# WojciechMula/pyahocorasick

Measured on NVIDIA H100. Metric: haystack GB/s, higher is better.
Workload: dtype u8

## Files before the change

### pyahocorasick_b200/csrc/acb_device.cu

```cuda
#include "acb_internal.h"
#include "acb_hash.h"

#include <cuda_runtime.h>
#include <cub/device/device_radix_sort.cuh>
#include <cub/device/device_scan.cuh>
#include <cub/device/device_select.cuh>

#include <algorithm>
#include <atomic>
#include <mutex>
#include <chrono>
#include <cstdio>
#include <cstdlib>
#include <cstring>
#include <exception>
#include <new>
#include <vector>

#define CUDA_TRY(expr)                                                                       \
    do {                                                                                     \
        cudaError_t _e = (expr);                                                             \
        if (_e != cudaSuccess) {                                                             \
            acb_set_error("CUDA error %s at %s:%d: %s", cudaGetErrorName(_e), __FILE__,      \
                          __LINE__, cudaGetErrorString(_e));                                 \
// ... 103 lines not shown
        hs = h * p.stride_bytes;
        he = hs + p.stride_bytes;
    } else {
        long long lo = 0, hi = p.n_hay;
        while (hi - lo > 1) {
            long long mid = (lo + hi) >> 1;
            if (__ldg(p.offsets + mid) <= q) lo = mid; else hi = mid;
        }
        h = lo;
        hs = __ldg(p.offsets + lo);
        he = __ldg(p.offsets + lo + 1);
    }
}

struct WarpStage {
    acb_match *buf;
    int *cnt;
};

__device__ __forceinline__ void emit(const ScanParams &p, const WarpStage &ws, int32_t h, int32_t e, int32_t k) {
    acb_match m;
    m.hay_id = h;
    m.end_index = e;
    m.key_id = k;
    int slot;
    asm volatile("atom.shared.add.u32 %0, [%1], 1;" : "=r"(slot) : "r"((uint32_t)__cvta_generic_to_shared(ws.cnt)) : "memory");
    if (slot < kStageCap) {
        ws.buf[slot] = m;
    } else {
        unsigned long long g = atomicAdd(p.count, 1ULL);
        if (g < (unsigned long long)p.cap) p.out[g] = m;
    }
}

__device__ __forceinline__ void flush_stage(const ScanParams &p, const WarpStage &ws, int lane) {
    __syncwarp();
    int n = *ws.cnt;
    if (n > kStageCap) n = kStageCap;
    if (n > 0) {
        unsigned long long base = 0;
        if (lane == 0) base = atomicAdd(p.count, (unsigned long long)n);
        base = __shfl_sync(kFull, base, 0);
#pragma unroll
        for (int i = lane; i < kStageCap; i += 32)
            if (i < n && base + i < (unsigned long long)p.cap) p.out[base + i] = ws.buf[i];
    }
    __syncwarp();
    if (lane == 0) *ws.cnt = 0;
    __syncwarp();
}

__device__ __forceinline__ void walk_from(const ScanParams &p, const WarpStage &ws, long long start,
                                          long long h, long long hs, long long he) {
    const int L = p.L;
    int32_t st = 0;
    for (long long i = start; i < he; ++i) {
        int c = __ldg(p.cls + p.hay[i]);
        int32_t nx = __ldg(p.gto + (long long)c * p.S + st);
        if (nx < 0) break;
        st = nx & kIdMask;
        if (nx & kTermBit) {
            int32_t k = __ldg(p.key_of + st);
            emit(p, ws, (int32_t)h, (int32_t)((i - hs + 1) / L - 1), k);
        }
    }
}

template <class P>
__device__ __forceinline__ void load_text(const P &p, long long x, uint32_t (&w)[6]) {
    const long long x0 = x & ~3LL;
    if (x0 + 24 <= p.total) {
        const uint32_t *a = reinterpret_cast<const uint32_t *>(p.hay + x0);
#pragma unroll
        for (int i = 0; i < 6; i++) w[i] = __ldg(a + i);
    } else {
#pragma unroll
        for (int i = 0; i < 6; i++) w[i] = load_word(p.hay, x0 + 4 * i, p.total);
    }
}

__device__ __forceinline__ bool text_equals(const uint32_t (&w)[6], long long x, int n, const uint32_t kw[5]) {
    const int sh = (int)(x & 3) * 8;
    uint32_t diff = 0;
#pragma unroll
    for (int i = 0; i < 5; i++) {
        uint32_t t = __funnelshift_r(w[i], w[i + 1], sh);
        int nb = n - 4 * i;
        uint32_t mask = nb >= 4 ? 0xffffffffu : (nb <= 0 ? 0u : ((1u << (8 * nb)) - 1u));
        diff |= (t ^ kw[i]) & mask;
    }
    return diff == 0;
}


__device__ __forceinline__ unsigned long long mul_wide(uint32_t a, uint32_t b) {
    unsigned long long d;
    asm("mul.wide.u32 %0, %1, %2;" : "=l"(d) : "r"(a), "r"(b));
    return d;
}
__device__ __forceinline__ unsigned long long mad_wide(uint32_t a, uint32_t b, unsigned long long c) {
    unsigned long long d;
    asm("mad.wide.u32 %0, %1, %2, %3;" : "=l"(d) : "r"(a), "r"(b), "l"(c));
    return d;
}
__device__ __forceinline__ uint32_t lds32(uint32_t saddr) {
    uint32_t v;
    asm volatile("ld.shared.u32 %0, [%1];" : "=r"(v) : "r"(saddr));
    return v;
}
__device__ __forceinline__ uint2 lds64(uint32_t saddr) {
    uint2 v;
    asm volatile("ld.shared.v2.u32 {%0, %1}, [%2];" : "=r"(v.x), "=r"(v.y) : "r"(saddr) : "memory");
    return v;
}
__device__ __forceinline__ uint32_t lds16(uint32_t saddr) {
    uint32_t v;
    asm volatile("{ .reg .u16 h; ld.shared.u16 h, [%1]; cvt.u32.u16 %0, h; }" : "=r"(v) : "r"(saddr) : "memory");
    return v;
}
__device__ __forceinline__ void sts16(uint32_t saddr, uint32_t v) {
    asm volatile("{ .reg .u16 h; cvt.u16.u32 h, %1; st.shared.u16 [%0], h; }" :: "r"(saddr), "r"(v) : "memory");
}
__device__ __forceinline__ uint4 lds128(uint32_t saddr) {
    uint4 v;
    asm volatile("ld.shared.v4.u32 {%0, %1, %2, %3}, [%4];" : "=r"(v.x), "=r"(v.y), "=r"(v.z), "=r"(v.w) : "r"(saddr));
    return v;
}
__device__ __forceinline__ uint32_t lds_bitmap(uint32_t saddr) {
    uint32_t v;
    asm("ld.shared.u32 %0, [%1];" : "=r"(v) : "r"(saddr));
    return v;
}

__device__ __forceinline__ void mbar_init(uint32_t bar, uint32_t count) {
    asm volatile("mbarrier.init.shared::cta.b64 [%0], %1;" :: "r"(bar), "r"(count) : "memory");
}
__device__ __forceinline__ void mbar_arrive(uint32_t bar) {
    asm volatile("mbarrier.arrive.shared::cta.b64 _, [%0];" :: "r"(bar) : "memory");
}
__device__ __forceinline__ void mbar_arrive_expect_tx(uint32_t bar, uint32_t bytes) {
    asm volatile("mbarrier.arrive.expect_tx.shared::cta.b64 _, [%0], %1;" :: "r"(bar), "r"(bytes) : "memory");
}
__device__ __forceinline__ void mbar_wait(uint32_t bar, uint32_t parity) {
    asm volatile(
        "{\n"
        ".reg .pred P1;\n"
        "LAB_WAIT:\n"
        "mbarrier.try_wait.parity.shared::cta.b64 P1, [%0], %1;\n"
        "@P1 bra DONE;\n"
        "bra LAB_WAIT;\n"
        "DONE:\n"
        "}" :: "r"(bar), "r"(parity) : "memory");
}
__device__ __forceinline__ void bulk_load(uint32_t dst, const void *src, uint32_t bytes, uint32_t bar) {
    asm volatile("cp.async.bulk.shared::cluster.global.mbarrier::complete_tx::bytes [%0], [%1], %2, [%3];"
                 :: "r"(dst), "l"(src), "r"(bytes), "r"(bar) : "memory");
}

__device__ __forceinline__ void resolve_chain(const ScanParams &p, const WarpStage &ws, long long q, uint32_t tag,
                                              const uint32_t (&tq)[6], uint4 e0, uint4 e1) {
    if (e0.x == 0u) return;
    long long h = -1, hs = 0, he = 0;
    if (e0.x == tag && (int32_t)e0.y >= 0 && (e0.z & 0x100ffu) == 0x10000u) {
        const uint32_t kw[5] = {e0.w, e1.x, e1.y, e1.z, e1.w};
        const int len = (int)((e0.z >> 8) & 0xffu);
        find_haystack(p, q, h, hs, he);
        if (q + len <= he && text_equals(tq, q, len, kw))
            emit(p, ws, (int32_t)h, (int32_t)(((q + len - hs) >> p.letter_shift) - 1), (int32_t)e0.y);
        return;
    }
    const uint32_t amask = (1u << p.logA) - 1u;
    uint32_t slot = tag >> (32 - p.logA);
    for (;;) {
        if (e0.x == 0u) break;
        if (e0.x == tag) {
            const uint32_t kw[5] = {e0.w, e1.x, e1.y, e1.z, e1.w};
            const int j = (int)(e0.z & 0xffu), len = (int)((e0.z >> 8) & 0xffu);
            const int32_t kid = (int32_t)e0.y;
            if (h < 0) find_haystack(p, q, h, hs, he);
            const long long start = q - j;
            if (start >= hs) {
                if (kid >= 0) {
                    bool eq = false;
                    if (start + len <= he) {
                        if (j == 0) eq = text_equals(tq, q, len, kw);
                        else { uint32_t ts[6]; load_text(p, start, ts); eq = text_equals(ts, start, len, kw); }
                    }
                    if (eq) emit(p, ws, (int32_t)h, (int32_t)(((start + len - hs) >> p.letter_shift) - 1), kid);
                } else if (q + len <= he && text_equals(tq, q, len, kw)) {
                    walk_from(p, ws, start, h, hs, he);
                }
            }
            if (e0.z & 0x10000u) break;
        }
        slot = (slot + 1) & amask;
        e0 = __ldg(p.anchors + 2 * (size_t)slot);
        e1 = __ldg(p.anchors + 2 * (size_t)slot + 1);
    }
}

struct ProbeCtx {
    uint32_t sbm;
    uint32_t n_words;
    uint32_t four;
    uint32_t two;
    int sh_bit;
};

template <int N>
__device__ __forceinline__ uint32_t window(const uint32_t (&W)[N], int t) {
    return ((t & 3) == 0) ? W[t >> 2] : __funnelshift_r(W[t >> 2], W[(t >> 2) + 1], (t & 3) * 8);
}

template <int NW, int STRIDE, bool WIDE>
__device__ __forceinline__ uint32_t probe_single(const ProbeCtx &c, const uint32_t (&W)[kLaneWords + NW], const uint32_t (&mul)[NW]) {
    constexpr int kProbes = kLaneBytes / STRIDE;
    uint32_t acc = 0;
#pragma unroll
    for (int t = 0; t < kLaneBytes; t += STRIDE) {
        uint32_t h = 0, ha;
        if (WIDE) {
            unsigned long long hw = 0;
#pragma unroll
            for (int k = 0; k < NW; k++) hw = mad_wide(window(W, t + 4 * k), mul[k], hw);
            h = (uint32_t)hw;
            ha = (uint32_t)(hw >> 32);
        } else {
#pragma unroll
            for (int k = 0; k < NW; k++) h += window(W, t + 4 * k) * mul[k];
            ha = h >> c.sh_bit;
        }
        const uint32_t word = lds_bitmap(__umulhi(h, c.n_words) * c.four + c.sbm);
        const uint32_t both = __funnelshift_r(word, 0u, ha) & __funnelshift_r(word, 0u, h) & 1u;
        acc = acc * c.two + both;
    }
    return __brev(acc) >> (32 - kProbes);
}

struct StreamSmem {
    uint32_t bitmap, stages, stage_rec, stage_cnt, bars, tiles, next, total;
};
__host__ __device__ inline StreamSmem stream_smem(int log1) {
    StreamSmem s;
    uint32_t o = 0;
    s.bitmap = o;    o += 1u << (log1 - 3);                       o = (o + 127u) & ~127u;
    s.stages = o;    o += (uint32_t)kStages * kStageBytes;
    s.stage_rec = o; o += (uint32_t)kConsumers * kStageCap * (uint32_t)sizeof(acb_match);
    s.stage_cnt = o; o += (uint32_t)kConsumers * 4u;              o = (o + 15u) & ~15u;
    s.bars = o;      o += 2u * kStages * 8u;
    s.tiles = o;     o += (uint32_t)kStages * 4u;
    s.next = o;      o += 4u;
    s.total = (o + 15u) & ~15u;
    return s;
}

__device__ __forceinline__ void resolve_backlog(const ScanParams &p, uint8_t *smem_raw, unsigned int n) {
    const int lane = threadIdx.x & 31, warp = threadIdx.x >> 5;
    const StreamSmem lay = stream_smem(p.log1);
    WarpStage ws;
    ws.buf = reinterpret_cast<acb_match *>(smem_raw + lay.stage_rec) + warp * kStageCap;
    ws.cnt = reinterpret_cast<int *>(smem_raw + lay.stage_cnt) + warp;
    const uint2 *list = p.cand + ((size_t)blockIdx.x * kConsumers + warp) * kWarpCand;
    __syncwarp();
    for (unsigned int i0 = 0; i0 < n; i0 += 32) {
        const unsigned int i = i0 + lane;
        if (i < n) {
            const uint2 e = __ldcg(list + i);
            const long long q = p.seg_begin + (long long)e.x;
            uint32_t tq[6];
            load_text(p, q, tq);
            const uint32_t slot = e.y >> (32 - p.logA);
            const uint4 a0 = __ldg(p.anchors + 2 * (size_t)slot), a1 = __ldg(p.anchors + 2 * (size_t)slot + 1);
            resolve_chain(p, ws, q, e.y, tq, a0, a1);
        }
        __syncwarp();
        if (*reinterpret_cast<volatile int *>(ws.cnt) >= kStageCap / 4) flush_stage(p, ws, lane);
    }
    flush_stage(p, ws, lane);
}

template <int NCONS, int TSLICES, int STAGES>
__device__ __forceinline__ void stream_producer(const ScanParams &p, uint8_t *smem_raw, uint32_t sbase, uint32_t stages,
                                                uint32_t bar_full, uint32_t bar_empty, volatile uint32_t *s_tile, int lane) {
    constexpr int kTileSlices = TSLICES, kStages = STAGES;
    constexpr int kTileBytes = kTileSlices * kSliceBytes;
    constexpr int kStageBytes = (kTileBytes + kLook + 127) / 128 * 128;
    struct { uint32_t stages; } lay = {stages};
    const uint8_t *seg = p.hay + p.seg_begin;
    const long long exist = p.total - p.seg_begin;
    unsigned int claim[kClaimDepth];
#pragma unroll
    for (int k = 0; k < kClaimDepth; k++) claim[k] = (lane == 0) ? atomicAdd(p.work_ctr, 1u) : 0u;
    bool more = true;
    for (uint32_t base = 0; more; base += kClaimDepth) {
#pragma unroll
        for (int k = 0; k < kClaimDepth; k++) {
            if (!more) break;
            const uint32_t fill = base + k;
            const uint32_t stage = fill % kStages;
            const unsigned int tile = __shfl_sync(kFull, claim[k], 0);
            if (lane == 0 && tile < p.n_tiles) claim[k] = atomicAdd(p.work_ctr, 1u);
            if (fill >= (uint32_t)kStages) mbar_wait(bar_empty + 8u * stage, ((fill / kStages) - 1u) & 1u);
            if (tile >= p.n_tiles) {
                constexpr uint32_t kSentinels = (NCONS + kTileSlices - 1) / kTileSlices;
                static_assert(kSentinels <= (uint32_t)kStages, "sentinel fills must not wrap the ring");
                for (uint32_t k2 = 0; k2 < kSentinels; k2++) {
                    const uint32_t f2 = fill + k2, st2 = f2 % kStages;
                    if (k2 > 0 && f2 >= (uint32_t)kStages) mbar_wait(bar_empty + 8u * st2, ((f2 / kStages) - 1u) & 1u);
                    if (lane == 0) { s_tile[st2] = kNoTile; mbar_arrive(bar_full + 8u * st2); }
                }
                more = false;
                break;
            }
            const long long off = (long long)tile * kTileBytes;
            const long long avail = exist - off;
            const uint32_t want = kTileBytes + kLook;
            const uint32_t bulk = avail >= (long long)want ? want : (uint32_t)(avail & ~15LL);
            uint8_t *dst = smem_raw + lay.stages + (size_t)stage * kStageBytes;
            if (avail < (long long)want) {
                const uint32_t a = (uint32_t)avail;
                uint32_t zend = ((a + (uint32_t)kSliceBytes - 1u) & ~((uint32_t)kSliceBytes - 1u)) + kLook;
                if (zend > want) zend = want;
                for (uint32_t i = bulk + lane; i < zend; i += 32) dst[i] = i < a ? seg[off + i] : (uint8_t)0;
                __syncwarp();
            }
            if (lane == 0) {
                s_tile[stage] = tile;
                if (bulk) {
                    mbar_arrive_expect_tx(bar_full + 8u * stage, bulk);
                    bulk_load(sbase + lay.stages + stage * (uint32_t)kStageBytes, seg + off, bulk, bar_full + 8u * stage);
                } else {
                    mbar_arrive(bar_full + 8u * stage);
                }
            }
        }
    }
    {
        unsigned int sink = 0;
#pragma unroll
        for (int k = 0; k < kClaimDepth; k++) sink |= claim[k];
        if (sink == 0x7fffffffu) s_tile[0] = sink;
    }
}

template <int NW, int STRIDE, int MODE>
__global__ void __launch_bounds__(kFThreads, 1) acb_stream_kernel(const __grid_constant__ ScanParams p) {
    extern __shared__ __align__(128) uint8_t smem_raw[];
    const StreamSmem lay = stream_smem(p.log1);
    const uint32_t sbase = (uint32_t)__cvta_generic_to_shared(smem_raw);
    const int tid = threadIdx.x, lane = tid & 31, warp = tid >> 5;
    const uint32_t bar_full = sbase + lay.bars, bar_empty = bar_full + 8u * kStages;
    volatile uint32_t *s_tile = reinterpret_cast<volatile uint32_t *>(smem_raw + lay.tiles);

    {
        const int n16 = 1 << (p.log1 - 7);
        const uint4 *src = reinterpret_cast<const uint4 *>(p.bm1);
        for (int i = tid; i < n16; i += kFThreads)
            asm volatile("cp.async.cg.shared.global [%0], [%1], 16;" :: "r"(sbase + lay.bitmap + 16u * i), "l"(src + i));
        asm volatile("cp.async.commit_group;");
        if (tid < kConsumers) reinterpret_cast<int *>(smem_raw + lay.stage_cnt)[tid] = 0;
        if (tid == 0) *reinterpret_cast<unsigned int *>(smem_raw + lay.next) = 0u;
        if (tid == 0) {
            for (int s = 0; s < kStages; s++) {
                mbar_init(bar_full + 8u * s, 1);
                mbar_init(bar_empty + 8u * s, kTileSlices);
            }
            asm volatile("fence.mbarrier_init.release.cluster;" ::: "memory");
        }
        asm volatile("cp.async.wait_group 0;" ::: "memory");
    }
    __syncthreads();

    const uint32_t seg_len = (uint32_t)(p.seg_end - p.seg_begin);

    if (warp == kConsumers) {
        stream_producer<kConsumers, kTileSlices, kStages>(p, smem_raw, sbase, lay.stages, bar_full, bar_empty, s_tile, lane);
    } else {
        ProbeCtx c;
        c.sbm = sbase + lay.bitmap;
        c.n_words = 1u << (p.log1 - 5);
        c.four = 4u + (uint32_t)(p.log1 >> 8);
        c.two = 2u + (uint32_t)(p.log1 >> 8);
        c.sh_bit = 32 - p.log1;
        const uint32_t lt_mask = (1u << lane) - 1u;
        uint32_t mul[NW];
#pragma unroll
        for (int k = 0; k < NW; k++) mul[k] = p.mul1[k];
        uint2 *list = p.cand + ((size_t)blockIdx.x * kConsumers + warp) * kWarpCand;
        uint32_t mul2[NW];
#pragma unroll
        for (int k = 0; k < NW; k++) mul2[k] = p.mul2[k];
        volatile uint16_t *items = reinterpret_cast<volatile uint16_t *>(smem_raw + lay.stage_rec + (size_t)warp * kStageCap * sizeof(acb_match));
        constexpr int kItemCap = kStageCap * (int)sizeof(acb_match) / 2;
        constexpr int kPendBits = kLaneBytes / STRIDE;
        unsigned int *s_next = reinterpret_cast<unsigned int *>(smem_raw + lay.next);
        unsigned int n_cand = 0;

        for (;;) {
            unsigned int g = 0;
            if (lane == 0) g = atomicAdd(s_next, 1u);
            g = __shfl_sync(kFull, g, 0);
            const uint32_t fill = g / (uint32_t)kTileSlices, slice_off = (g % (uint32_t)kTileSlices) * (uint32_t)kSliceBytes;
            const uint32_t stage = fill % (uint32_t)kStages;
            mbar_wait(bar_full + 8u * stage, (fill / (uint32_t)kStages) & 1u);
            const uint32_t tile = s_tile[stage];
            if (tile == kNoTile) break;
            const uint32_t tile_off = tile * (uint32_t)kTileBytes;
            const uint32_t n_valid = (seg_len - tile_off < (uint32_t)kTileBytes) ? seg_len - tile_off : (uint32_t)kTileBytes;
            if (slice_off < n_valid) {
                const uint32_t slice_saddr = sbase + lay.stages + stage * (uint32_t)kStageBytes + slice_off;
                const uint32_t saddr = slice_saddr + (uint32_t)lane * kLaneBytes;
                uint32_t W[kLaneWords + NW];
#pragma unroll
                for (int i = 0; i < kLaneWords; i += 4) {
                    const uint4 v = lds128(saddr + 4u * i);
                    W[i] = v.x; W[i + 1] = v.y; W[i + 2] = v.z; W[i + 3] = v.w;
                }
#pragma unroll
                for (int k = 0; k < NW; k++) W[kLaneWords + k] = __shfl_down_sync(kFull, W[k], 1);
                if (lane == 31) {
#pragma unroll
                    for (int k = 0; k < NW; k++) W[kLaneWords + k] = lds32(saddr + kLaneBytes + 4u * k);
                }
                uint32_t pend;
#ifdef ACB_EXP_NOPROBE
                pend = (W[0] ^ W[3] ^ W[kLaneWords]) == 0x12345678u ? 1u : 0u;
#else
                pend = probe_single<NW, STRIDE, MODE == kModeWide>(c, W, mul);
#endif
                if (n_valid - slice_off < (uint32_t)kSliceBytes) {
                    const int v = (int)(n_valid - slice_off) - lane * kLaneBytes;
                    const int valid = (v + STRIDE - 1) / STRIDE;
                    pend = (valid <= 0) ? 0u : ((valid >= 32) ? pend : (pend & ((1u << valid) - 1u)));
                }
#ifdef ACB_EXP_NOSURV
                if (pend == 0x9e3779b9u) s_tile[0] = 1u;
                pend = 0;
#endif
                if (__ballot_sync(kFull, pend != 0)) {
                    const unsigned int total = __reduce_add_sync(kFull, (unsigned int)__popc(pend));
                    const int nparts = (total > (unsigned int)kItemCap && kPendBits > 8) ? kPendBits / 8 : 1;
                    for (int part = 0; part < nparts; part++) {
                        uint32_t m = nparts > 1 ? ((pend >> (8 * part)) & 0xffu) : pend;
                        const int cnt = __popc(m);
                        int incl = cnt;
#pragma unroll
                        for (int d = 1; d < 32; d <<= 1) {
                            const int v = __shfl_up_sync(kFull, incl, d);
                            if (lane >= d) incl += v;
                        }
                        const int tot = __shfl_sync(kFull, incl, 31);
                        int at = incl - cnt;
                        while (m) {
                            const int bit = __ffs(m) - 1;
                            m &= m - 1;
                            items[at++] = (uint16_t)((lane << 5) | (bit + (nparts > 1 ? 8 * part : 0)));
                        }
                        __syncwarp();
                        for (int base = 0; base < tot; base += 32) {
                            bool ok0 = false;
                            uint32_t pos0 = 0, tag0 = 0;
                            if (base + lane < tot) {
                                const uint32_t it = items[base + lane];
                                const uint32_t t = (it >> 5) * (uint32_t)kLaneBytes + (it & 31u) * (uint32_t)STRIDE;
                                const uint32_t ga = slice_saddr + t, wa = ga & ~3u, sh = (ga & 3u) * 8u;
                                pos0 = tile_off + slice_off + t;
                                {
                                    uint32_t w0 = lds32(wa);
#pragma unroll
                                    for (int k = 0; k < NW; k++) {
                                        const uint32_t w1 = lds32(wa + 4u * (k + 1));
                                        tag0 += __funnelshift_r(w0, w1, sh) * mul2[k];
                                        w0 = w1;
                                    }
                                    tag0 |= 1u;
                                    ok0 = true;
                                }
                            }
                            if (p.log3) {
                                const uint32_t i0 = (tag0 * ACB_TAGMAP_MIX) >> (32 - p.log3);
                                if (ok0) ok0 = ((__ldg(p.bm3 + (i0 >> 5)) >> (i0 & 31u)) & 1u) != 0u;
                            }
#ifndef ACB_EXP_NODRAIN
                            const unsigned m0 = __ballot_sync(kFull, ok0);
                            if (ok0) list[n_cand + __popc(m0 & lt_mask)] = make_uint2(pos0, tag0);
                            n_cand += __popc(m0);
#else
                            if (ok0 && tag0 == pos0) s_tile[0] = 2u;
#endif
                        }
                        __syncwarp();
                    }
                }
            }
            __syncwarp();
            if (lane == 0) mbar_arrive(bar_empty + 8u * stage);
            if (n_cand >= 32u) { resolve_backlog(p, smem_raw, n_cand); n_cand = 0; }
        }
        if (n_cand) resolve_backlog(p, smem_raw, n_cand);
    }
    __syncthreads();
    if (tid == 0) {
        __threadfence();
        unsigned int done = atomicAdd(p.work_ctr + 1, 1u);
        if (done == gridDim.x - 1) {
            p.work_ctr[0] = 0u;
            p.work_ctr[1] = 0u;
            __threadfence();
        }
    }
}

#ifndef ACB_PAIR_CONSUMERS
#define ACB_PAIR_CONSUMERS 27
#endif
constexpr int kPairConsumers = ACB_PAIR_CONSUMERS;
constexpr int kPairThreads = (kPairConsumers + 1) * 32;
#ifndef ACB_PAIR_TILE_SLICES
#define ACB_PAIR_TILE_SLICES 32
#endif
#ifndef ACB_PAIR_STAGES
#define ACB_PAIR_STAGES 2
#endif
constexpr int kPairTileSlices = ACB_PAIR_TILE_SLICES;
constexpr int kPairStages     = ACB_PAIR_STAGES;
constexpr int kPairTileLog    = __builtin_ctz(kPairTileSlices);
constexpr int kPairStageLog   = __builtin_ctz(kPairStages);
constexpr int kPairTileBytes  = kPairTileSlices * kSliceBytes;
constexpr int kPairStageBytes = (kPairTileBytes + kLook + 127) / 128 * 128;
static_assert((kPairTileSlices & (kPairTileSlices - 1)) == 0 && (kPairStages & (kPairStages - 1)) == 0 && kSliceBytes == 1024,
              "pair ring: power-of-two tiles and stages of 1 KiB slices");
static_assert((kPairConsumers + kPairTileSlices - 1) / kPairTileSlices + 2 < 2 * kPairStages && kPairThreads <= 1024, "pair kernel shape");
constexpr int kPairRing = 64;
constexpr int kPairItems = 64;
static_assert(kPairRing >= 31 + 32, "a one-round slice must fit the ring next to a turn not yet resolved");

struct PairTurnArgs {
    const uint8_t *hay;
    long long total;
    long long seg_begin;
    const uint4 *anchors;
    int logA, stride_shift, letter_shift, pad;
    const long long *offsets;
    long long n_hay;
    long long stride_bytes;
    long long cap;
    acb_match *out;
    unsigned long long *count;
};
static_assert(sizeof(PairTurnArgs) == 96, "PairTurnArgs is six 16-byte groups");

struct PairSmem {
    uint32_t bitmap, bitmap2, stages, ring, items, args, bars, tiles, next, total;
};
__host__ __device__ inline PairSmem pair_smem(int log1, int log2b) {
    PairSmem s;
    uint32_t o = 0;
    s.bitmap = o;    o += 1u << (log1 - 3);
    s.bitmap2 = o;   o += 1u << (log2b - 3);                      o = (o + 127u) & ~127u;
    s.stages = o;    o += (uint32_t)kPairStages * kPairStageBytes;
    s.ring = o;      o += (uint32_t)kPairConsumers * kPairRing * 8u;
    s.items = o;     o += (uint32_t)kPairConsumers * kPairItems * 2u;
    s.bars = o;      o += 2u * kPairStages * 8u;
    s.tiles = o;     o += (uint32_t)kPairStages * 4u;
    s.next = o;      o += 4u;                                     o = (o + 15u) & ~15u;
    s.args = o;      o += (uint32_t)sizeof(PairTurnArgs);
    s.total = o;
    return s;
}

__device__ __forceinline__ void emit_direct(const ScanParams &p, int32_t h, int32_t e, int32_t k) {
    const unsigned long long g = atomicAdd(p.count, 1ULL);
    if (g < (unsigned long long)p.cap) { acb_match m; m.hay_id = h; m.end_index = e; m.key_id = k; p.out[g] = m; }
}

__device__ __noinline__ void pair_resolve_general(const ScanParams &p, long long q, uint32_t tag, uint32_t slot, uint4 e0, uint4 e1) {
    const uint32_t amask = (1u << p.logA) - 1u;
    long long h = -1, hs = 0, he = 0;
    for (;;) {
        if (e0.x == 0u) break;
        if (e0.x == tag) {
            const uint32_t kw[5] = {e0.w, e1.x, e1.y, e1.z, e1.w};
            const int j = (int)(e0.z & 0xffu), len = (int)((e0.z >> 8) & 0xffu);
            const int32_t kid = (int32_t)e0.y;
            if (h < 0) find_haystack(p, q, h, hs, he);
            const long long start = q - j;
            if (start >= hs && start + len <= he) {
                uint32_t ts[6];
                load_text(p, start, ts);
                if (text_equals(ts, start, len, kw)) {
                    if (kid >= 0) {
                        emit_direct(p, (int32_t)h, (int32_t)(((start + len - hs) >> p.letter_shift) - 1), kid);
                    } else {
                        int32_t st = 0;
                        for (long long i = start; i < he; ++i) {
                            const int c = __ldg(p.cls + p.hay[i]);
                            const int32_t nx = __ldg(p.gto + (long long)c * p.S + st);
                            if (nx < 0) break;
                            st = nx & kIdMask;
                            if (nx & kTermBit) emit_direct(p, (int32_t)h, (int32_t)((i - hs + 1) / p.L - 1), __ldg(p.key_of + st));
                        }
                    }
                }
            }
            if (e0.z & 0x10000u) break;
        }
        slot = (slot + 1) & amask;
        e0 = __ldg(p.anchors + 2 * (size_t)slot);
        e1 = __ldg(p.anchors + 2 * (size_t)slot + 1);
    }
}

union PairTurnRegs {
    uint4 v[sizeof(PairTurnArgs) / 16];
    PairTurnArgs a;
};
__device__ __forceinline__ void load_turn_args(PairTurnRegs &u, int g0, int g1) {
    extern __shared__ __align__(128) uint8_t smem_raw[];
    uint32_t dyn;
    asm("mov.u32 %0, %%dynamic_smem_size;" : "=r"(dyn));
    const uint32_t saddr = (uint32_t)__cvta_generic_to_shared(smem_raw) + dyn - (uint32_t)sizeof(PairTurnArgs);
#pragma unroll
    for (int i = g0; i < g1; i++)
        asm("ld.shared.v4.u32 {%0, %1, %2, %3}, [%4];" : "=r"(u.v[i].x), "=r"(u.v[i].y), "=r"(u.v[i].z), "=r"(u.v[i].w) : "r"(saddr + 16u * i));
}

__device__ __noinline__ void pair_resolve(const ScanParams &p, uint32_t sring, unsigned int head, unsigned int n) {
    const int lane = threadIdx.x & 31;
    const uint32_t lt_mask = (1u << lane) - 1u;
    PairTurnRegs u;
    const PairTurnArgs &a = u.a;
    bool hit = false;
    int32_t rh = 0, re = 0, rk = 0;
    if ((unsigned)lane < n) {
        load_turn_args(u, 0, 3);
        const uint32_t amask = (1u << a.logA) - 1u;
        const uint2 e = lds64(sring + (((head + (unsigned)lane) & (kPairRing - 1u)) << 3));
        const long long q = a.seg_begin + (long long)e.x;
        uint32_t slot = e.y >> (32 - a.logA);
        uint4 e0 = __ldg(a.anchors + 2 * (size_t)slot), e1 = __ldg(a.anchors + 2 * (size_t)slot + 1);
        uint32_t tq[6];
        load_text(a, q, tq);
        while (e0.x != 0u && e0.x != e.y) {
            slot = (slot + 1) & amask;
            e0 = __ldg(a.anchors + 2 * (size_t)slot);
            e1 = __ldg(a.anchors + 2 * (size_t)slot + 1);
        }
        if (e0.x != 0u) {
            if ((int32_t)e0.y >= 0 && (e0.z & 0x100ffu) == 0x10000u) {
                const uint32_t kw[5] = {e0.w, e1.x, e1.y, e1.z, e1.w};
                const int len = (int)((e0.z >> 8) & 0xffu);
                long long h, hs, he;
                load_turn_args(u, 3, 5);
                find_haystack(a, q, h, hs, he);
                hit = q + len <= he && text_equals(tq, q, len, kw);
                rh = (int32_t)h;
                re = (int32_t)(((q + len - hs) >> a.letter_shift) - 1);
                rk = (int32_t)e0.y;
            } else {
                pair_resolve_general(p, q, e.y, slot, e0, e1);
            }
        }
    }
    load_turn_args(u, 4, 6);
    const unsigned mh = __ballot_sync(kFull, hit);
    if (mh) {
        unsigned long long base = 0;
        if (lane == 0)
            asm volatile("atom.global.add.u64 %0, [%1], %2;" : "=l"(base) : "l"(__cvta_generic_to_global(a.count)), "l"((unsigned long long)__popc(mh)) : "memory");
        base = __shfl_sync(kFull, base, 0) + (unsigned long long)__popc(mh & lt_mask);
        if (hit && base < (unsigned long long)a.cap)
            asm volatile("st.global.u32 [%0], %1;\n\tst.global.u32 [%0+4], %2;\n\tst.global.u32 [%0+8], %3;"
                         :: "l"(__cvta_generic_to_global(a.out + base)), "r"(rh), "r"(re), "r"(rk) : "memory");
    }
}

__device__ __forceinline__ uint32_t probe_pair_run(uint32_t acc, uint32_t sbm, uint32_t n_words, uint32_t four, const uint32_t (&R)[5], uint32_t mulp) {
#pragma unroll
    for (int x = 0; x < 16; x += 2) {
#ifdef ACB_EXP_L1_NOWIDE
        const uint32_t hc = window(R, x + 1) * mulp, hb = hc >> 7;
#else
        const unsigned long long pr = mul_wide(window(R, x + 1), mulp);
        const uint32_t hc = (uint32_t)pr, hb = (uint32_t)(pr >> 32);
#endif
#ifdef ACB_EXP_L1_SHIFTIDX
        const uint32_t waddr = (hc >> 17) * four + sbm;
#else
        const uint32_t waddr = __umulhi(hc, n_words) * four + sbm;
#endif
#ifdef ACB_EXP_L1_NOLDS
        const uint32_t word = waddr;
#else
        const uint32_t word = lds_bitmap(waddr);
#endif
        const uint32_t ta = __funnelshift_l(0u, word, window(R, x));
        const uint32_t tb = __funnelshift_l(0u, word, hb);
#ifdef ACB_L1_CARRY
        asm("{ .reg .u32 t2; add.cc.u32 t2, %1, %1; addc.u32 %0, %0, %0; add.cc.u32 t2, %2, %2; addc.u32 %0, %0, %0; }"
            : "+r"(acc) : "r"(ta), "r"(tb));
#else
        acc = __funnelshift_l(ta, acc, 1);
        acc = __funnelshift_l(tb, acc, 1);
#endif
    }
    return acc;
}

template <int L2B>
__global__ void __launch_bounds__(kPairThreads, 1) acb_pair_kernel(const __grid_constant__ ScanParams p) {
    extern __shared__ __align__(128) uint8_t smem_raw[];
    const PairSmem lay = pair_smem(p.log1, p.log2b);
    const uint32_t sbase = (uint32_t)__cvta_generic_to_shared(smem_raw);
    const int tid = threadIdx.x, lane = tid & 31, warp = tid >> 5;
    const uint32_t bar_full = sbase + lay.bars, bar_empty = bar_full + 8u * kPairStages;
    volatile uint32_t *s_tile = reinterpret_cast<volatile uint32_t *>(smem_raw + lay.tiles);

    if (tid == 0) {
        *reinterpret_cast<unsigned int *>(smem_raw + lay.next) = 0u;
        PairTurnArgs &a = *reinterpret_cast<PairTurnArgs *>(smem_raw + lay.args);
        a.hay = p.hay; a.total = p.total; a.seg_begin = p.seg_begin; a.anchors = p.anchors;
        a.logA = p.logA; a.stride_shift = p.stride_shift; a.letter_shift = p.letter_shift; a.pad = 0;
        a.offsets = p.offsets; a.n_hay = p.n_hay; a.stride_bytes = p.stride_bytes; a.cap = p.cap;
        a.out = p.out; a.count = p.count;
        for (int s = 0; s < kPairStages; s++) {
            mbar_init(bar_full + 8u * s, 1);
            mbar_init(bar_empty + 8u * s, kPairTileSlices);
        }
        asm volatile("fence.mbarrier_init.release.cluster;" ::: "memory");
    }
    __syncthreads();

    const uint32_t seg_len = (uint32_t)(p.seg_end - p.seg_begin);

    if (warp == kPairConsumers) {
        stream_producer<kPairConsumers, kPairTileSlices, kPairStages>(p, smem_raw, sbase, lay.stages, bar_full, bar_empty, s_tile, lane);
    } else {
        {
            const int n16 = (1 << (p.log1 - 7)) + (1 << (p.log2b - 7));
            const uint4 *src = reinterpret_cast<const uint4 *>(p.bm1);
            for (int i = tid; i < n16; i += kPairConsumers * 32)
                asm volatile("cp.async.cg.shared.global [%0], [%1], 16;" :: "r"(sbase + lay.bitmap + 16u * i), "l"(src + i));
            asm volatile("cp.async.commit_group;");
            asm volatile("cp.async.wait_group 0;" ::: "memory");
            asm volatile("bar.sync 1, %0;" :: "n"(kPairConsumers * 32) : "memory");
        }
        const uint32_t sbm = sbase + lay.bitmap, sbm2 = sbase + lay.bitmap2;
        const uint32_t n_words = 1u << (p.log1 - 5);
        const int l2b = L2B ? L2B : p.log2b;
        const int shy_w = 37 - l2b, shy_a = 32 - l2b, shy_b = 27 - l2b;
        const uint32_t four = 4u + (uint32_t)(p.log1 >> 8);
        const uint32_t mulp = acb_pair_mul() + (uint32_t)(p.log1 >> 8);
        const uint32_t mul2 = p.mul2[0];
        const uint32_t lt_mask = (1u << lane) - 1u;
        const uint32_t sring = sbase + lay.ring + (uint32_t)warp * (kPairRing * 8u);
        const uint32_t sitems = sbase + lay.items + (uint32_t)warp * (kPairItems * 2u);
        const uint32_t snext = sbase + lay.next;
        const uint32_t sstages = sbase + lay.stages;
        const uint32_t lane16 = (uint32_t)lane << 4;
        unsigned int n_cand = 0, head = 0;

        auto offset_of = [&](uint32_t y) { return lane16 + y + (y & 16u) * 31u; };
        auto top_bit = [](uint32_t m) { uint32_t y; asm("bfind.u32 %0, %1;" : "=r"(y) : "r"(m)); return y; };
        auto list_all = [&](uint32_t pend) {
            const unsigned int cnt = (unsigned)__popc(pend);
            unsigned int incl = cnt;
#pragma unroll
            for (int d = 1; d < 32; d <<= 1) {
                const unsigned int v = __shfl_up_sync(kFull, incl, d);
                if (lane >= d) incl += v;
            }
            uint32_t at = sitems + 2u * (incl - cnt);
            while (pend) {
                const uint32_t y = top_bit(pend);
                pend ^= 1u << y;
                sts16(at, offset_of(y));
                at += 2u;
            }
        };
        auto item_round = [&](uint32_t slice_saddr, uint32_t pos_base, unsigned int base, unsigned int take) {
            uint32_t ok = 0, pos = 0, tag = 0;
            if ((unsigned)lane < take) {
                const uint32_t t = lds16(sitems + 2u * (base + (unsigned)lane));
                const uint32_t ga = slice_saddr + t, wa = ga & ~3u;
                const uint32_t lo = lds32(wa), hi = lds32(wa + 4u);
                const uint32_t w = __funnelshift_r(lo, hi, ga << 3);
                tag = (w * mul2) | 1u;
                const uint32_t word = lds_bitmap((tag >> shy_w) * four + sbm2);
                ok = __funnelshift_r(word, 0u, tag >> shy_a) & __funnelshift_r(word, 0u, tag >> shy_b) & 1u;
                pos = pos_base + t;
            }
            if (p.log3) {
                const uint32_t i0 = (tag * ACB_TAGMAP_MIX) >> (32 - p.log3);
                if (ok) ok = (__ldg(p.bm3 + (i0 >> 5)) >> (i0 & 31u)) & 1u;
            }
#ifdef ACB_EXP_NODRAIN
            if (ok && tag == pos) s_tile[0] = 2u;
#else
            const unsigned mk = __ballot_sync(kFull, ok);
            if (ok) {
                const uint32_t at = sring + (((head + n_cand + (unsigned)__popc(mk & lt_mask)) & (kPairRing - 1u)) << 3);
                asm volatile("st.shared.v2.u32 [%0], {%1, %2};" :: "r"(at), "r"(pos), "r"(tag) : "memory");
            }
            n_cand += (unsigned)__popc(mk);
#endif
        };

        for (;;) {
            unsigned int g = 0;
            asm volatile("{ .reg .pred e; elect.sync _|e, 0xffffffff; @e atom.shared.add.u32 %0, [%1], 1; }"
                         : "+r"(g) : "r"(snext) : "memory");
            g = __shfl_sync(kFull, g, 0);
            const uint32_t fill = g >> kPairTileLog, stage = fill & (kPairStages - 1u);
            const uint32_t slice_off = (g & (kPairTileSlices - 1u)) * (uint32_t)kSliceBytes;
            mbar_wait(bar_full + 8u * stage, (fill >> kPairStageLog) & 1u);
            const uint32_t tile = s_tile[stage];
            if (tile == kNoTile) break;
            const uint32_t tile_off = tile * (uint32_t)kPairTileBytes;
            const uint32_t n_valid = (seg_len - tile_off < (uint32_t)kPairTileBytes) ? seg_len - tile_off : (uint32_t)kPairTileBytes;
            const uint32_t slice_saddr = sstages + stage * (uint32_t)kPairStageBytes + slice_off;
            const uint32_t pos_base = tile_off + slice_off;
            uint32_t pend = 0;
            if (slice_off < n_valid) {
                const uint32_t saddr = slice_saddr + lane16;
                uint32_t R0[5], R1[5];
                {
                    const uint4 v = lds128(saddr), u = lds128(saddr + 512u);
                    R0[0] = v.x; R0[1] = v.y; R0[2] = v.z; R0[3] = v.w;
                    R1[0] = u.x; R1[1] = u.y; R1[2] = u.z; R1[3] = u.w;
                }
                R0[4] = __shfl_down_sync(kFull, R0[0], 1);
                R1[4] = __shfl_down_sync(kFull, R1[0], 1);
                const uint32_t r1_first = __shfl_sync(kFull, R1[0], 0);
                if (lane == 31) { R0[4] = r1_first; R1[4] = lds32(slice_saddr + (uint32_t)kSliceBytes); }
#ifdef ACB_EXP_NOPROBE
                pend = (R0[0] ^ R0[3] ^ R0[4] ^ R1[1] ^ R1[4]) == 0x12345678u ? 1u : 0u;
#else
                pend = probe_pair_run(0u, sbm, n_words, four, R0, mulp);
                pend = probe_pair_run(pend, sbm, n_words, four, R1, mulp);
                pend = __brev(pend);
#endif
                if (n_valid - slice_off < (uint32_t)kSliceBytes) {
                    const int v0 = (int)(n_valid - slice_off) - lane * 16, v1 = v0 - 512;
                    const uint32_t m0 = v0 <= 0 ? 0u : (v0 >= 16 ? 0xffffu : ((1u << v0) - 1u));
                    const uint32_t m1 = v1 <= 0 ? 0u : (v1 >= 16 ? 0xffffu : ((1u << v1) - 1u));
                    pend &= m0 | (m1 << 16);
                }
#ifdef ACB_EXP_NOSURV
                if (pend == 0x9e3779b9u) s_tile[0] = 1u;
                pend = 0;
#endif
            }
            unsigned int tot = __reduce_add_sync(kFull, (unsigned)__popc(pend));
            if (tot <= 32u) {
                if (tot) {
                    list_all(pend);
                    __syncwarp();
                    item_round(slice_saddr, pos_base, 0u, tot);
                }
            } else {
                while (tot) {
                    unsigned int n_items;
                    if (tot <= (unsigned)kPairItems) {
                        list_all(pend);
                        n_items = tot;
                        tot = 0;
                    } else {
                        n_items = 0;
                        do {
                            const unsigned int mp = __ballot_sync(kFull, pend != 0u);
                            if (pend) {
                                const uint32_t y = top_bit(pend);
                                pend ^= 1u << y;
                                sts16(sitems + 2u * (n_items + (unsigned)__popc(mp & lt_mask)), offset_of(y));
                            }
                            n_items += (unsigned)__popc(mp);
                        } while (n_items <= (unsigned)(kPairItems - 32));
                        tot -= n_items;
                    }
                    __syncwarp();
                    for (unsigned int base = 0; base < n_items;) {
                        if (n_cand == (unsigned)kPairRing) {
                            __syncwarp();
                            pair_resolve(p, sring, head, 32u); head += 32u; n_cand -= 32u;
                            continue;
                        }
                        unsigned int take = n_items - base;
                        if (take > 32u) take = 32u;
                        if (take > (unsigned)kPairRing - n_cand) take = (unsigned)kPairRing - n_cand;
                        item_round(slice_saddr, pos_base, base, take);
                        base += take;
                    }
                    __syncwarp();
                }
            }
            __syncwarp();
            if (lane == 0) mbar_arrive(bar_empty + 8u * stage);
            while (n_cand >= 32u) { pair_resolve(p, sring, head, 32u); head += 32u; n_cand -= 32u; }
        }
        if (n_cand) { __syncwarp(); pair_resolve(p, sring, head, n_cand); }
    }
    __syncthreads();
    if (tid == 0) {
        __threadfence();
        unsigned int done = atomicAdd(p.work_ctr + 1, 1u);
        if (done == gridDim.x - 1) {
            p.work_ctr[0] = 0u;
            p.work_ctr[1] = 0u;
            __threadfence();
        }
    }
}


__global__ void __launch_bounds__(kDfaThreads) acb_dfa_kernel(const ScanParams p) {
    const long long span = (long long)blockIdx.x * blockDim.x + threadIdx.x;
    const long long a = span * kDfaSpan;
    if (a >= p.total) return;
    const long long b = (a + kDfaSpan < p.total) ? a + kDfaSpan : p.total;
    long long h, hs, he;
    find_haystack(p, a, h, hs, he);
    long long i = a - p.max_key_bytes;
    if (i < hs) i = hs;
    int32_t st = 0;
    const int L = p.L;
    for (; i < b; ++i) {
        while (i >= he) {
            h += 1; hs = he;
            he = (p.offsets == nullptr) ? hs + p.stride_bytes : __ldg(p.offsets + h + 1);
            st = 0;
        }
        const long long col = (long long)__ldg(p.cls + p.hay[i]) * p.S;
        int32_t nx;
        while ((nx = __ldg(p.gto + col + st)) < 0 && st != 0) st = __ldg(p.fail + st);
        st = (nx < 0) ? 0 : (nx & kIdMask);
        if (i >= a && st != 0 && ((i + 1 - hs) % L) == 0) {
            const int32_t o0 = __ldg(p.out_ptr + st), o1 = __ldg(p.out_ptr + st + 1);
            for (int32_t o = o0; o < o1; ++o) {
                const int32_t k = __ldg(p.out_idx + o);
                const long long kb = (long long)__ldg(p.key_len + k) * L;
                if (i + 1 - kb < hs) continue;
                unsigned long long g = atomicAdd(p.count, 1ULL);
                if (g < (unsigned long long)p.cap) {
                    acb_match m;
                    m.hay_id = (int32_t)h;
                    m.end_index = (int32_t)((i - hs + 1) / L - 1);
                    m.key_id = k;
                    p.out[g] = m;
                }
            }
        }
    }
}

__device__ __forceinline__ int32_t letter_step(const ScanParams &p, int32_t st, const uint8_t *letter) {
    for (int b = 0; b < p.L; b++) {
        const int32_t nx = __ldg(p.gto + (long long)__ldg(p.cls + letter[b]) * p.S + st);
        if (nx < 0) return -1;
        st = nx & kIdMask;
    }
    return st;
}

__global__ void __launch_bounds__(kDfaThreads) acb_long_kernel(const __grid_constant__ ScanParams p) {
    const long long h = (long long)blockIdx.x * blockDim.x + threadIdx.x;
    if (h >= p.n_hay) return;
    const long long hs = p.offsets ? __ldg(p.offsets + h) : h * p.stride_bytes;
    const long long he = p.offsets ? __ldg(p.offsets + h + 1) : hs + p.stride_bytes;
    const long long n = (he - hs) / p.L;
    const uint8_t *text = p.hay + hs;
    int32_t state = p.long_start ? __ldg(p.long_start + h) : ((h == 0) ? p.long_init : 0), last_node = -1;
    long long index = -1, last_index = -1;
    for (;;) {
        if (last_node >= 0) {
            unsigned long long g = atomicAdd(p.count, 1ULL);
            if (g < (unsigned long long)p.cap) {
                acb_match m;
                m.hay_id = (int32_t)h;
                m.end_index = (int32_t)last_index;
                m.key_id = __ldg(p.key_of + last_node);
                p.out[g] = m;
            }
            state = 0;
            index = last_index;
            last_node = -1;
            last_index = -1;
        }
        index += 1;
        bool emit = false;
        while (index < n) {
            const int32_t nx = letter_step(p, state, text + index * p.L);
            if (nx >= 0) {
                if (__ldg(p.key_of + nx) >= 0) {
                    last_node = nx;
                    last_index = index;
                } else {
                    const int32_t fl = __ldg(p.letter_fail + nx);
                    if (fl > 0 && __ldg(p.key_of + fl) >= 0) { last_node = fl; last_index = index; emit = true; break; }
                }
                state = nx;
                index += 1;
            } else {
                if (last_node >= 0) { emit = true; break; }
                for (;;) {
                    state = __ldg(p.letter_fail + state);
                    if (state < 0) { state = 0; index += 1; break; }
                    if (letter_step(p, state, text + index * p.L) >= 0) break;
                }
            }
        }
        if (!emit && last_node < 0) break;
    }
    if (h == 0 && p.long_final) *p.long_final = state;
    if (p.long_end) p.long_end[h] = state;
}

__global__ void acb_flag_goto_kernel(int32_t *gto, const int32_t *key_of, size_t n) {
    for (size_t i = (size_t)blockIdx.x * blockDim.x + threadIdx.x; i < n; i += (size_t)gridDim.x * blockDim.x) {
        const int32_t v = gto[i];
        if (v >= 0 && key_of[v] >= 0) gto[i] = v | kTermBit;
    }
}

}


struct acb_table {
    int device = 0;
    int sm_count = 0;
    int32_t S = 0, K = 0, L = 1, n_keys = 0, gram = 1, stride = 1, log1 = 13, log3 = 0, logA = 10, filter_flags = 0, log2b = 0;
    int32_t min_key_bytes = 0, max_key_bytes = 0;
    uint32_t mul1[ACB_MAX_WINDOWS], mul2[ACB_MAX_WINDOWS];
    uint8_t *d_cls = nullptr;
    int32_t *d_lfail = nullptr;
    int32_t *d_goto = nullptr, *d_fail = nullptr, *d_keyof = nullptr, *d_outptr = nullptr, *d_outidx = nullptr, *d_keylen = nullptr;
    uint32_t *d_bm1 = nullptr, *d_bm3 = nullptr, *d_anchors = nullptr;
    unsigned int *d_work = nullptr;
    uint2 *d_cand = nullptr;
    int32_t long_init = 0;
    int32_t *d_long_final = nullptr;
    int32_t long_final_host = -1;
    long long dev_bytes = 0;
    std::vector<int32_t> key_len;
    cudaStream_t stream = nullptr, s_copy = nullptr, s_sort = nullptr;
    std::vector<cudaEvent_t> ev_h2d, ev_scan;
    unsigned long long *h_counts = nullptr; size_t h_counts_cap = 0;
    cudaEvent_t ev0 = nullptr, ev1 = nullptr;
    uint8_t *w_hay = nullptr; size_t w_hay_cap = 0;
    long long *w_off = nullptr; size_t w_off_cap = 0;
    acb_match *w_out = nullptr; size_t w_out_cap = 0;
// ... 2879 lines not shown
```

Baseline: 1468.

## Process two-slice units per consumer turn and poll fill counters before mbarrier

Consumer warps now claim 2 KiB units (two slices) per turn instead of one slice, halving the shared-counter atomics and empty-barrier arrivals per tile. A per-stage fill counter, published with a release store by the producer, is polled with nanosleep before the mbarrier parity wait, so consumers that claimed a future fill do not wait on the wrong phase. Item rounds now drain the candidate ring on demand rather than capping each round's take. This changes load balance granularity and adds per-turn register and latency cost from the larger unit.

After: 1343 (median of 6 runs). 8.5% lower.

```diff
diff --git a/pyahocorasick_b200/csrc/acb_device.cu b/pyahocorasick_b200/csrc/acb_device.cu
--- a/pyahocorasick_b200/csrc/acb_device.cu
+++ b/pyahocorasick_b200/csrc/acb_device.cu
@@ -279,6 +279,27 @@
         "DONE:\n"
         "}" :: "r"(bar), "r"(parity) : "memory");
 }
+__device__ __forceinline__ void st_release_shared(volatile uint32_t *p, uint32_t v) {
+    asm volatile("st.release.cta.shared.u32 [%0], %1;" :: "r"((uint32_t)__cvta_generic_to_shared((const void *)p)), "r"(v) : "memory");
+}
+template <int SLOG>
+__device__ __forceinline__ void fill_wait(uint32_t sfill, uint32_t bar, uint32_t fill) {
+    asm volatile(
+        "{\n"
+        ".reg .pred P1;\n"
+        ".reg .b32 f, ph;\n"
+        "LAB_FILL:\n"
+        "ld.acquire.cta.shared.u32 f, [%0];\n"
+        "setp.ne.u32 P1, f, %2;\n"
+        "@P1 nanosleep.u32 32;\n"
+        "@P1 bra LAB_FILL;\n"
+        "shr.b32 ph, %2, %3;\n"
+        "and.b32 ph, ph, 1;\n"
+        "LAB_PHASE:\n"
+        "mbarrier.try_wait.parity.shared::cta.b64 P1, [%1], ph;\n"
+        "@!P1 bra LAB_PHASE;\n"
+        "}" :: "r"(sfill), "r"(bar), "r"(fill), "n"(SLOG) : "memory");
+}
 __device__ __forceinline__ void bulk_load(uint32_t dst, const void *src, uint32_t bytes, uint32_t bar) {
     asm volatile("cp.async.bulk.shared::cluster.global.mbarrier::complete_tx::bytes [%0], [%1], %2, [%3];"
                  :: "r"(dst), "l"(src), "r"(bytes), "r"(bar) : "memory");
@@ -406,7 +427,7 @@
     flush_stage(p, ws, lane);
 }
 
-template <int NCONS, int TSLICES, int STAGES>
+template <int NCONS, int TSLICES, int STAGES, int TUNITS = TSLICES, bool FILLS = false>
 __device__ __forceinline__ void stream_producer(const ScanParams &p, uint8_t *smem_raw, uint32_t sbase, uint32_t stages,
                                                 uint32_t bar_full, uint32_t bar_empty, volatile uint32_t *s_tile, int lane) {
     constexpr int kTileSlices = TSLICES, kStages = STAGES;
@@ -429,12 +450,16 @@
             if (lane == 0 && tile < p.n_tiles) claim[k] = atomicAdd(p.work_ctr, 1u);
             if (fill >= (uint32_t)kStages) mbar_wait(bar_empty + 8u * stage, ((fill / kStages) - 1u) & 1u);
             if (tile >= p.n_tiles) {
-                constexpr uint32_t kSentinels = (NCONS + kTileSlices - 1) / kTileSlices;
+                constexpr uint32_t kSentinels = (NCONS + TUNITS - 1) / TUNITS;
                 static_assert(kSentinels <= (uint32_t)kStages, "sentinel fills must not wrap the ring");
                 for (uint32_t k2 = 0; k2 < kSentinels; k2++) {
                     const uint32_t f2 = fill + k2, st2 = f2 % kStages;
                     if (k2 > 0 && f2 >= (uint32_t)kStages) mbar_wait(bar_empty + 8u * st2, ((f2 / kStages) - 1u) & 1u);
-                    if (lane == 0) { s_tile[st2] = kNoTile; mbar_arrive(bar_full + 8u * st2); }
+                    if (lane == 0) {
+                        s_tile[st2] = kNoTile;
+                        if (FILLS) st_release_shared(s_tile + kStages + st2, f2);
+                        mbar_arrive(bar_full + 8u * st2);
+                    }
                 }
                 more = false;
                 break;
@@ -453,6 +478,7 @@
             }
             if (lane == 0) {
                 s_tile[stage] = tile;
+                if (FILLS) st_release_shared(s_tile + kStages + stage, fill);
                 if (bulk) {
                     mbar_arrive_expect_tx(bar_full + 8u * stage, bulk);
                     bulk_load(sbase + lay.stages + stage * (uint32_t)kStageBytes, seg + off, bulk, bar_full + 8u * stage);
@@ -651,16 +677,18 @@
 #endif
 constexpr int kPairTileSlices = ACB_PAIR_TILE_SLICES;
 constexpr int kPairStages     = ACB_PAIR_STAGES;
-constexpr int kPairTileLog    = __builtin_ctz(kPairTileSlices);
+constexpr int kPairUnitBytes  = 2 * kSliceBytes;
+constexpr int kPairTileUnits  = kPairTileSlices / 2;
+constexpr int kPairUnitLog    = __builtin_ctz(kPairTileUnits);
 constexpr int kPairStageLog   = __builtin_ctz(kPairStages);
 constexpr int kPairTileBytes  = kPairTileSlices * kSliceBytes;
 constexpr int kPairStageBytes = (kPairTileBytes + kLook + 127) / 128 * 128;
-static_assert((kPairTileSlices & (kPairTileSlices - 1)) == 0 && (kPairStages & (kPairStages - 1)) == 0 && kSliceBytes == 1024,
-              "pair ring: power-of-two tiles and stages of 1 KiB slices");
-static_assert((kPairConsumers + kPairTileSlices - 1) / kPairTileSlices + 2 < 2 * kPairStages && kPairThreads <= 1024, "pair kernel shape");
+static_assert(kPairTileSlices >= 2 && (kPairTileSlices & (kPairTileSlices - 1)) == 0 && (kPairStages & (kPairStages - 1)) == 0 &&
+              kSliceBytes == 1024, "pair ring: power-of-two tiles (of at least one unit) and stages of 1 KiB slices");
+static_assert(kPairThreads <= 1024, "pair kernel shape");
 constexpr int kPairRing = 64;
 constexpr int kPairItems = 64;
-static_assert(kPairRing >= 31 + 32, "a one-round slice must fit the ring next to a turn not yet resolved");
+static_assert(kPairRing >= 32 + 32, "a round's survivors must fit the ring next to what one turn leaves");
 
 struct PairTurnArgs {
     const uint8_t *hay;
@@ -677,6 +705,7 @@
 };
 static_assert(sizeof(PairTurnArgs) == 96, "PairTurnArgs is six 16-byte groups");
 
+constexpr uint32_t kPairFillsOff = 2u * kPairStages * 8u + kPairStages * 4u;
 struct PairSmem {
     uint32_t bitmap, bitmap2, stages, ring, items, args, bars, tiles, next, total;
 };
@@ -689,7 +718,7 @@
     s.ring = o;      o += (uint32_t)kPairConsumers * kPairRing * 8u;
     s.items = o;     o += (uint32_t)kPairConsumers * kPairItems * 2u;
     s.bars = o;      o += 2u * kPairStages * 8u;
-    s.tiles = o;     o += (uint32_t)kPairStages * 4u;
+    s.tiles = o;     o += 2u * kPairStages * 4u;
     s.next = o;      o += 4u;                                     o = (o + 15u) & ~15u;
     s.args = o;      o += (uint32_t)sizeof(PairTurnArgs);
     s.total = o;
@@ -852,7 +881,8 @@
         a.out = p.out; a.count = p.count;
         for (int s = 0; s < kPairStages; s++) {
             mbar_init(bar_full + 8u * s, 1);
-            mbar_init(bar_empty + 8u * s, kPairTileSlices);
+            mbar_init(bar_empty + 8u * s, kPairTileUnits);
+            s_tile[kPairStages + s] = 0xffffffffu;
         }
         asm volatile("fence.mbarrier_init.release.cluster;" ::: "memory");
     }
@@ -861,7 +891,7 @@
     const uint32_t seg_len = (uint32_t)(p.seg_end - p.seg_begin);
 
     if (warp == kPairConsumers) {
-        stream_producer<kPairConsumers, kPairTileSlices, kPairStages>(p, smem_raw, sbase, lay.stages, bar_full, bar_empty, s_tile, lane);
+        stream_producer<kPairConsumers, kPairTileSlices, kPairStages, kPairTileUnits, true>(p, smem_raw, sbase, lay.stages, bar_full, bar_empty, s_tile, lane);
     } else {
         {
             const int n16 = (1 << (p.log1 - 7)) + (1 << (p.log2b - 7));
@@ -889,8 +919,8 @@
 
         auto offset_of = [&](uint32_t y) { return lane16 + y + (y & 16u) * 31u; };
         auto top_bit = [](uint32_t m) { uint32_t y; asm("bfind.u32 %0, %1;" : "=r"(y) : "r"(m)); return y; };
-        auto list_all = [&](uint32_t pend) {
-            const unsigned int cnt = (unsigned)__popc(pend);
+        auto list_all = [&](uint32_t pend0, uint32_t pend1) {
+            const unsigned int cnt = (unsigned)(__popc(pend0) + __popc(pend1));
             unsigned int incl = cnt;
 #pragma unroll
             for (int d = 1; d < 32; d <<= 1) {
@@ -898,18 +928,24 @@
                 if (lane >= d) incl += v;
             }
             uint32_t at = sitems + 2u * (incl - cnt);
-            while (pend) {
-                const uint32_t y = top_bit(pend);
-                pend ^= 1u << y;
+            while (pend0) {
+                const uint32_t y = top_bit(pend0);
+                pend0 ^= 1u << y;
                 sts16(at, offset_of(y));
                 at += 2u;
             }
+            while (pend1) {
+                const uint32_t y = top_bit(pend1);
+                pend1 ^= 1u << y;
+                sts16(at, offset_of(y) + (uint32_t)kSliceBytes);
+                at += 2u;
+            }
         };
-        auto item_round = [&](uint32_t slice_saddr, uint32_t pos_base, unsigned int base, unsigned int take) {
+        auto item_round = [&](uint32_t unit_saddr, uint32_t pos_base, unsigned int base, unsigned int take) {
             uint32_t ok = 0, pos = 0, tag = 0;
             if ((unsigned)lane < take) {
                 const uint32_t t = lds16(sitems + 2u * (base + (unsigned)lane));
-                const uint32_t ga = slice_saddr + t, wa = ga & ~3u;
+                const uint32_t ga = unit_saddr + t, wa = ga & ~3u;
                 const uint32_t lo = lds32(wa), hi = lds32(wa + 4u);
                 const uint32_t w = __funnelshift_r(lo, hi, ga << 3);
                 tag = (w * mul2) | 1u;
@@ -925,12 +961,43 @@
             if (ok && tag == pos) s_tile[0] = 2u;
 #else
             const unsigned mk = __ballot_sync(kFull, ok);
+            const unsigned int n_ok = (unsigned)__popc(mk);
+            if (n_cand + n_ok > (unsigned)kPairRing) {
+                __syncwarp();
+                pair_resolve(p, sring, head, 32u); head += 32u; n_cand -= 32u;
+            }
             if (ok) {
                 const uint32_t at = sring + (((head + n_cand + (unsigned)__popc(mk & lt_mask)) & (kPairRing - 1u)) << 3);
                 asm volatile("st.shared.v2.u32 [%0], {%1, %2};" :: "r"(at), "r"(pos), "r"(tag) : "memory");
             }
-            n_cand += (unsigned)__popc(mk);
+            n_cand += n_ok;
 #endif
+        };
+        auto level1 = [&](uint32_t half_saddr) -> uint32_t {
+            const uint32_t saddr = half_saddr + lane16;
+            uint32_t R0[5], R1[5];
+            {
+                const uint4 v = lds128(saddr), u = lds128(saddr + 512u);
+                R0[0] = v.x; R0[1] = v.y; R0[2] = v.z; R0[3] = v.w;
+                R1[0] = u.x; R1[1] = u.y; R1[2] = u.z; R1[3] = u.w;
+            }
+            R0[4] = __shfl_down_sync(kFull, R0[0], 1);
+            R1[4] = __shfl_down_sync(kFull, R1[0], 1);
+            const uint32_t r1_first = __shfl_sync(kFull, R1[0], 0);
+            if (lane == 31) { R0[4] = r1_first; R1[4] = lds32(half_saddr + (uint32_t)kSliceBytes); }
+#ifdef ACB_EXP_NOPROBE
+            return (R0[0] ^ R0[3] ^ R0[4] ^ R1[1] ^ R1[4]) == 0x12345678u ? 1u : 0u;
+#else
+            uint32_t acc = probe_pair_run(0u, sbm, n_words, four, R0, mulp);
+            acc = probe_pair_run(acc, sbm, n_words, four, R1, mulp);
+            return __brev(acc);
+#endif
+        };
+        auto valid_mask = [&](int v) {
+            const int v0 = v - lane * 16, v1 = v0 - 512;
+            const uint32_t m0 = v0 <= 0 ? 0u : (v0 >= 16 ? 0xffffu : ((1u << v0) - 1u));
+            const uint32_t m1 = v1 <= 0 ? 0u : (v1 >= 16 ? 0xffffu : ((1u << v1) - 1u));
+            return m0 | (m1 << 16);
         };
 
         for (;;) {
@@ -938,91 +1005,74 @@
             asm volatile("{ .reg .pred e; elect.sync _|e, 0xffffffff; @e atom.shared.add.u32 %0, [%1], 1; }"
                          : "+r"(g) : "r"(snext) : "memory");
             g = __shfl_sync(kFull, g, 0);
-            const uint32_t fill = g >> kPairTileLog, stage = fill & (kPairStages - 1u);
-            const uint32_t slice_off = (g & (kPairTileSlices - 1u)) * (uint32_t)kSliceBytes;
-            mbar_wait(bar_full + 8u * stage, (fill >> kPairStageLog) & 1u);
+            const uint32_t fill = g >> kPairUnitLog, stage = fill & (kPairStages - 1u);
+            const uint32_t unit_off = (g & (kPairTileUnits - 1u)) * (uint32_t)kPairUnitBytes;
+            fill_wait<kPairStageLog>(bar_full + kPairFillsOff + 4u * stage, bar_full + 8u * stage, fill);
             const uint32_t tile = s_tile[stage];
             if (tile == kNoTile) break;
             const uint32_t tile_off = tile * (uint32_t)kPairTileBytes;
             const uint32_t n_valid = (seg_len - tile_off < (uint32_t)kPairTileBytes) ? seg_len - tile_off : (uint32_t)kPairTileBytes;
-            const uint32_t slice_saddr = sstages + stage * (uint32_t)kPairStageBytes + slice_off;
-            const uint32_t pos_base = tile_off + slice_off;
-            uint32_t pend = 0;
-            if (slice_off < n_valid) {
-                const uint32_t saddr = slice_saddr + lane16;
-                uint32_t R0[5], R1[5];
-                {
-                    const uint4 v = lds128(saddr), u = lds128(saddr + 512u);
-                    R0[0] = v.x; R0[1] = v.y; R0[2] = v.z; R0[3] = v.w;
-                    R1[0] = u.x; R1[1] = u.y; R1[2] = u.z; R1[3] = u.w;
-                }
-                R0[4] = __shfl_down_sync(kFull, R0[0], 1);
-                R1[4] = __shfl_down_sync(kFull, R1[0], 1);
-                const uint32_t r1_first = __shfl_sync(kFull, R1[0], 0);
-                if (lane == 31) { R0[4] = r1_first; R1[4] = lds32(slice_saddr + (uint32_t)kSliceBytes); }
-#ifdef ACB_EXP_NOPROBE
-                pend = (R0[0] ^ R0[3] ^ R0[4] ^ R1[1] ^ R1[4]) == 0x12345678u ? 1u : 0u;
-#else
-                pend = probe_pair_run(0u, sbm, n_words, four, R0, mulp);
-                pend = probe_pair_run(pend, sbm, n_words, four, R1, mulp);
-                pend = __brev(pend);
-#endif
-                if (n_valid - slice_off < (uint32_t)kSliceBytes) {
-                    const int v0 = (int)(n_valid - slice_off) - lane * 16, v1 = v0 - 512;
-                    const uint32_t m0 = v0 <= 0 ? 0u : (v0 >= 16 ? 0xffffu : ((1u << v0) - 1u));
-                    const uint32_t m1 = v1 <= 0 ? 0u : (v1 >= 16 ? 0xffffu : ((1u << v1) - 1u));
-                    pend &= m0 | (m1 << 16);
+            const uint32_t unit_saddr = sstages + stage * (uint32_t)kPairStageBytes + unit_off;
+            const uint32_t pos_base = tile_off + unit_off;
+            uint32_t pend0 = 0, pend1 = 0;
+            if (unit_off < n_valid) {
+                const uint32_t n_here = n_valid - unit_off;
+                pend0 = level1(unit_saddr);
+                if (n_here > (uint32_t)kSliceBytes) pend1 = level1(unit_saddr + (uint32_t)kSliceBytes);
+                if (n_here < (uint32_t)kPairUnitBytes) {
+                    pend0 &= valid_mask((int)n_here);
+                    pend1 &= valid_mask((int)n_here - kSliceBytes);
                 }
 #ifdef ACB_EXP_NOSURV
-                if (pend == 0x9e3779b9u) s_tile[0] = 1u;
-                pend = 0;
+                if ((pend0 ^ pend1) == 0x9e3779b9u) s_tile[0] = 1u;
+                pend0 = pend1 = 0;
 #endif
             }
-            unsigned int tot = __reduce_add_sync(kFull, (unsigned)__popc(pend));
-            if (tot <= 32u) {
+            unsigned int tot = __reduce_add_sync(kFull, (unsigned)(__popc(pend0) + __popc(pend1)));
+            if (tot <= (unsigned)kPairItems) {
                 if (tot) {
-                    list_all(pend);
+                    list_all(pend0, pend1);
                     __syncwarp();
-                    item_round(slice_saddr, pos_base, 0u, tot);
+                    item_round(unit_saddr, pos_base, 0u, tot < 32u ? tot : 32u);
+                    if (tot > 32u) item_round(unit_saddr, pos_base, 32u, tot - 32u);
                 }
             } else {
-                while (tot) {
+                do {
                     unsigned int n_items;
                     if (tot <= (unsigned)kPairItems) {
-                        list_all(pend);
+                        list_all(pend0, pend1);
+                        pend0 = pend1 = 0;
                         n_items = tot;
-                        tot = 0;
                     } else {
                         n_items = 0;
                         do {
-                            const unsigned int mp = __ballot_sync(kFull, pend != 0u);
-                            if (pend) {
-                                const uint32_t y = top_bit(pend);
-                                pend ^= 1u << y;
-                                sts16(sitems + 2u * (n_items + (unsigned)__popc(mp & lt_mask)), offset_of(y));
+                            const bool has = (pend0 | pend1) != 0u;
+                            const unsigned int mp = __ballot_sync(kFull, has);
+                            if (has) {
+                                uint32_t off;
+                                if (pend0) {
+                                    const uint32_t y = top_bit(pend0);
+                                    pend0 ^= 1u << y;
+                                    off = offset_of(y);
+                                } else {
+                                    const uint32_t y = top_bit(pend1);
+                                    pend1 ^= 1u << y;
+                                    off = offset_of(y) + (uint32_t)kSliceBytes;
+                                }
+                                sts16(sitems + 2u * (n_items + (unsigned)__popc(mp & lt_mask)), off);
                             }
                             n_items += (unsigned)__popc(mp);
                         } while (n_items <= (unsigned)(kPairItems - 32));
-                        tot -= n_items;
                     }
                     __syncwarp();
-                    for (unsigned int base = 0; base < n_items;) {
-                        if (n_cand == (unsigned)kPairRing) {
-                            __syncwarp();
-                            pair_resolve(p, sring, head, 32u); head += 32u; n_cand -= 32u;
-                            continue;
-                        }
-                        unsigned int take = n_items - base;
-                        if (take > 32u) take = 32u;
-                        if (take > (unsigned)kPairRing - n_cand) take = (unsigned)kPairRing - n_cand;
-                        item_round(slice_saddr, pos_base, base, take);
-                        base += take;
-                    }
+                    for (unsigned int base = 0; base < n_items; base += 32u)
+                        item_round(unit_saddr, pos_base, base, n_items - base < 32u ? n_items - base : 32u);
                     __syncwarp();
-                }
+                    tot = __reduce_add_sync(kFull, (unsigned)(__popc(pend0) + __popc(pend1)));
+                } while (tot);
             }
             __syncwarp();
-            if (lane == 0) mbar_arrive(bar_empty + 8u * stage);
+            if (lane == 0) mbar_arrive(bar_empty + 8u * ((unit_saddr - sstages) / (uint32_t)kPairStageBytes));
             while (n_cand >= 32u) { pair_resolve(p, sring, head, 32u); head += 32u; n_cand -= 32u; }
         }
         if (n_cand) { __syncwarp(); pair_resolve(p, sring, head, n_cand); }
```
